# Complexity-ML/complexity-tokenizer

Hardware: AMD Instinct MI355X
Metric: MB/s raw UTF-8 encoded (encode_batch), 50k ByteLevel BPE, 1/2/4/8 MI355X (higher is better)
Workload: dtype u8

## Files before the change

complexity-tokenizer_amd/csrc/seg_lane.h:

```cpp
#pragma once
#include <cstdint>

#if defined(__HIP_DEVICE_COMPILE__)
#define SEG_HD __device__ __forceinline__
#else
#define SEG_HD inline
#endif

namespace seg {

constexpr uint32_t kHi = 0x80808080u;
constexpr uint32_t rep(uint32_t c) { return c * 0x01010101u; }

SEG_HD uint32_t mulhi(uint32_t a, uint32_t b) {
#if defined(__HIP_DEVICE_COMPILE__)
  return __umulhi(a, b);
#else
  return (uint32_t)(((uint64_t)a * b) >> 32);
#endif
}

SEG_HD uint32_t pack8(uint32_t r0, uint32_t r1) {
  const uint32_t c = ((r0 & kHi) >> 4) | (r1 & kHi);
  return mulhi(c, 0x20408100u) & 0xFFu;
}

SEG_HD uint32_t ne7(uint32_t x7, uint32_t c) {
  const uint32_t t = x7 ^ rep(c);
  return (t + 0x7F7F7F7Fu) | t;
}
SEG_HD uint32_t in80(uint32_t x80, uint32_t lo, uint32_t hi) {
  return (x80 - rep(lo)) & ~(x80 - rep(hi + 1));
}

struct Masks {
  uint64_t W, L, N, S, Q, NA;
};
struct Letters {
  uint64_t T1, R, Le, V, LL;
};

SEG_HD Masks ascii_masks(const uint32_t (&x)[16]) {
  uint32_t w[2] = {0, 0}, l[2] = {0, 0}, n[2] = {0, 0}, s[2] = {0, 0}, q[2] = {0, 0}, na[2] = {0, 0};
#pragma unroll
  for (int p = 0; p < 8; p++) {
    const uint32_t a = x[2 * p], b = x[2 * p + 1];
    const uint32_t a7 = a & 0x7F7F7F7Fu, b7 = b & 0x7F7F7F7Fu;
    const uint32_t a80 = a | kHi, b80 = b | kHi;
    const int h = p >> 2, sh = 8 * (p & 3);
    s[h] |= pack8(ne7(a7, ' '), ne7(b7, ' ')) << sh;
    q[h] |= pack8(ne7(a7, '\''), ne7(b7, '\'')) << sh;
    w[h] |= pack8(in80(a80, 9, 13), in80(b80, 9, 13)) << sh;
    l[h] |= pack8(in80(a80 | rep(0x20), 'a', 'z'), in80(b80 | rep(0x20), 'a', 'z')) << sh;
    n[h] |= pack8(in80(a80, '0', '9'), in80(b80, '0', '9')) << sh;
    na[h] |= pack8(a, b) << sh;
  }
  Masks m;
  m.NA = (uint64_t)na[0] | ((uint64_t)na[1] << 32);
  m.S = ~((uint64_t)s[0] | ((uint64_t)s[1] << 32)) & ~m.NA;
  m.Q = ~((uint64_t)q[0] | ((uint64_t)q[1] << 32)) & ~m.NA;
  m.W = (((uint64_t)w[0] | ((uint64_t)w[1] << 32)) | m.S) & ~m.NA;
  m.L = ((uint64_t)l[0] | ((uint64_t)l[1] << 32)) & ~m.NA;
  m.N = ((uint64_t)n[0] | ((uint64_t)n[1] << 32)) & ~m.NA;
  return m;
}

SEG_HD Letters letter_masks(const uint32_t (&x)[16], uint64_t na) {
  uint32_t t1[2] = {0, 0}, r[2] = {0, 0}, e[2] = {0, 0}, v[2] = {0, 0}, ll[2] = {0, 0};
#pragma unroll
  for (int p = 0; p < 8; p++) {
    const uint32_t a7 = x[2 * p] & 0x7F7F7F7Fu, b7 = x[2 * p + 1] & 0x7F7F7F7Fu;
    const int h = p >> 2, sh = 8 * (p & 3);
    t1[h] |= pack8(ne7(a7, 's') & ne7(a7, 't') & ne7(a7, 'm') & ne7(a7, 'd'),
                   ne7(b7, 's') & ne7(b7, 't') & ne7(b7, 'm') & ne7(b7, 'd')) << sh;
    r[h] |= pack8(ne7(a7, 'r'), ne7(b7, 'r')) << sh;
    e[h] |= pack8(ne7(a7, 'e'), ne7(b7, 'e')) << sh;
    v[h] |= pack8(ne7(a7, 'v'), ne7(b7, 'v')) << sh;
    ll[h] |= pack8(ne7(a7, 'l'), ne7(b7, 'l')) << sh;
  }
  auto inv = [&](const uint32_t (&y)[2]) { return ~((uint64_t)y[0] | ((uint64_t)y[1] << 32)) & ~na; };
  return Letters{inv(t1), inv(r), inv(e), inv(v), inv(ll)};
}

SEG_HD uint64_t p1(uint64_t c, uint64_t p) { return (c << 1) | (p >> 63); }
SEG_HD uint64_t p2(uint64_t c, uint64_t p) { return (c << 2) | (p >> 62); }
SEG_HD uint64_t p3(uint64_t c, uint64_t p) { return (c << 3) | (p >> 61); }
SEG_HD uint64_t n1(uint64_t c, uint64_t n) { return (c >> 1) | (n << 63); }
SEG_HD uint64_t n2(uint64_t c, uint64_t n) { return (c >> 2) | (n << 62); }

SEG_HD uint64_t attached(const Masks& c, uint64_t D, uint64_t pW, uint64_t nW, uint64_t nD) {
  const uint64_t E = n1(D, nD);
  return c.S & ~E & ~n1(c.W, nW) & (D | ~p1(c.W, pW));
}

SEG_HD void contractions(const Masks& c, const Letters& lt, uint64_t D, uint64_t A, uint64_t pA, uint64_t pP,
                         uint64_t nL, uint64_t nD, const Letters& nl, uint64_t& C1, uint64_t& C2) {
  const uint64_t E = n1(D, nD);
  const uint64_t P = ~(c.W | c.L | c.N);
  const uint64_t Cb = c.Q & ~E & n1(c.L, nL) & (D | (~p1(P, pP) & ~p1(A, pA)));
  const uint64_t t1 = n1(lt.T1, nl.T1);
  C1 = Cb & t1;
  C2 = Cb & ~t1 & ~n2(D, nD) &
       (((n1(lt.R, nl.R) | n1(lt.V, nl.V)) & n2(lt.Le, nl.Le)) | (n1(lt.LL, nl.LL) & n2(lt.LL, nl.LL)));
}

SEG_HD uint64_t starts(const Masks& c, uint64_t D, uint64_t pW, uint64_t pL, uint64_t pN, uint64_t A, uint64_t pA,
                       uint64_t C1, uint64_t C2, uint64_t pC1, uint64_t pC2) {
  const uint64_t chg = (c.W ^ p1(c.W, pW)) | (c.L ^ p1(c.L, pL)) | (c.N ^ p1(c.N, pN));
  return D | (chg & ~p1(A, pA) & ~p1(C1 | C2, pC1 | pC2)) | (~chg & c.L & (p2(C1, pC1) | p3(C2, pC2)));
}

}
```

complexity-tokenizer_amd/csrc/segment.hip:

```cpp
#include "dev_common.h"
#include "seg_lane.h"

namespace ctok_dev {


__global__ __launch_bounds__(256) void k_tilefirst(const uint64_t* __restrict__ off, uint32_t n_docs, uint32_t n_tiles,
                                                   uint32_t* __restrict__ tfirst, uint32_t* __restrict__ counters) {
  const uint32_t d = blockIdx.x * blockDim.x + threadIdx.x;
  bool empty = false;
  if (d <= n_docs && n_tiles) {
    const uint64_t y = off[d];
    empty = d < n_docs && y == off[d + 1];
    const uint64_t t_lo = d ? (off[d - 1] + 64) / kTile + 1 : 0ull;
    const uint64_t t_hi = min((y + 64) / kTile, (uint64_t)n_tiles - 1);
    for (uint64_t t = t_lo; t <= t_hi && t < t_lo + 64; t++) tfirst[t] = d;
  } else if (d < n_docs) {
    empty = off[d] == off[d + 1];
  }
  const uint64_t me = __ballot(empty);
  if (me && (threadIdx.x & 63) == (uint32_t)__ffsll((unsigned long long)me) - 1)
    atomicAdd(&counters[kCtrEmptyDocs], (uint32_t)__popcll(me));
}

__device__ uint32_t tile_first_search(const uint64_t* off, uint32_t n_docs, uint32_t tile) {
  const uint64_t key = tile ? (uint64_t)tile * kTile - 64 : 0ull;
  uint32_t lo = 0, hi = n_docs;
  while (lo < hi) {
    const uint32_t mid = lo + (hi - lo) / 2;
    if (__builtin_amdgcn_readfirstlane((uint32_t)(off[mid] < key))) lo = mid + 1;
    else hi = mid;
  }
  return lo;
}

__device__ __forceinline__ void clear_words(uint32_t* __restrict__ p, uint64_t n) {
  const uint64_t n4 = n / 4;
  uint4* p4 = reinterpret_cast<uint4*>(p);
  for (uint64_t i = (uint64_t)blockIdx.x * 256 + threadIdx.x; i < n4; i += (uint64_t)gridDim.x * 256)
    p4[i] = make_uint4(0u, 0u, 0u, 0u);
  if (blockIdx.x == 0 && threadIdx.x < n - 4 * n4) p[4 * n4 + threadIdx.x] = 0u;
}

__global__ __launch_bounds__(256) void k_clear(uint32_t* __restrict__ bits, uint64_t n, uint32_t* __restrict__ counters,
                                               uint32_t* __restrict__ tfirst, uint32_t n_tiles) {
  if (bits) clear_words(bits, n);
  for (uint32_t i = blockIdx.x * 256 + threadIdx.x; i < n_tiles; i += gridDim.x * 256) tfirst[i] = ~0u;
  if (blockIdx.x == 0 && counters && threadIdx.x < (uint32_t)kCounterWords) counters[threadIdx.x] = 0u;
}

uint64_t nfc_bits_words(uint64_t n_bytes) { return (n_bytes + 2047) / 2048 + 8; }

hipError_t launch_docstart(const Work& w, hipStream_t s, bool zero_counters, Lx x, Lx x2) {
  const bool nfc = w.nfc_watch == 2;
  const uint64_t n = nfc ? nfc_bits_words(w.n_bytes) : 0;
  const uint64_t work = std::max<uint64_t>(n / 4, w.n_tiles);
  launch_lx(x, k_clear, (unsigned)std::min<uint64_t>((work + 255) / 256 + 1, 8ull * w.n_cus), 256, 0, s,
            nfc ? w.nfc_bits : nullptr, n, zero_counters ? w.counters : nullptr, w.tfirst, w.n_tiles);
  if (w.n_tiles) launch_lx(x2, k_tilefirst, (w.n_docs + 1 + 255) / 256, 256, 0, s, w.doc_off, w.n_docs, w.n_tiles, w.tfirst, w.counters);
  else if (w.n_docs)
    k_tilefirst<<<(w.n_docs + 255) / 256, 256, 0, s>>>(w.doc_off, w.n_docs, 0, w.tfirst, w.counters);
  return hipGetLastError();
}


__device__ __forceinline__ uint32_t piece_probe(const Tables& t, uint4 e, uint32_t h, uint32_t lo, uint32_t hi,
                                                uint32_t n) {
  while (e.z != 0) {
    if (e.x == lo && e.y == hi && e.z == n) return e.w;
    h = (h + 1) & t.piece_mask;
    e = t.piece_tab[h];
  }
  return kNone;
}

__device__ __forceinline__ void seg_wave_sync() {
  __builtin_amdgcn_fence(__ATOMIC_RELEASE, "wavefront");
  __builtin_amdgcn_wave_barrier();
  __builtin_amdgcn_fence(__ATOMIC_ACQUIRE, "wavefront");
}

__device__ __forceinline__ uint32_t select_bit(uint64_t x, uint32_t k) {
  uint32_t pos = 0;
  uint32_t lo = (uint32_t)x, hi = (uint32_t)(x >> 32);
  uint32_t c = __popc(lo);
  uint32_t v = lo;
  if (k >= c) { k -= c; v = hi; pos = 32; }
#pragma unroll
  for (int wdt = 16; wdt >= 1; wdt >>= 1) {
    const uint32_t m = (1u << wdt) - 1u;
    c = __popc(v & m);
    if (k >= c) { k -= c; v >>= wdt; pos += wdt; }
  }
  return pos;
}




#ifdef CTOK_SEG_STAMPS
#define SEG_STAMP(k)                                                                              \
  do {                                                                                            \
    __builtin_amdgcn_sched_barrier(0);                                                            \
    unsigned long long t_;                                                                        \
    asm volatile("s_memtime %0\n\ts_waitcnt lgkmcnt(0)" : "=s"(t_)::"memory");                     \
    __builtin_amdgcn_sched_barrier(0);                                                            \
    if (w.stamps && lane == 0) w.stamps[(size_t)tile * 8 + (k)] = t_;                            \
  } while (0)
#else
#define SEG_STAMP(k) do { } while (0)
#endif
template <bool R16>
__global__ __launch_bounds__(64 * kSegWaves) __attribute__((amdgpu_waves_per_eu(7))) void k_segment(Work w, Tables t) {
  __shared__ uint16_t s_pos_all[kSegWaves][64 * kSegUnroll + 8];
  __shared__ __attribute__((aligned(16))) uint32_t s_text_all[kSegWaves][(kTileWords + 2) * 16 + 8];
  __shared__ uint64_t s_D_all[kSegWaves][64];
  constexpr uint32_t kSegLongCap = 32;
  __shared__ uint64_t s_long_all[kSegWaves][kSegLongCap];
  __shared__ uint8_t s_buf_all[kSegWaves][kSegListBuf];
  const uint32_t lane = threadIdx.x & 63;
  const uint32_t wid = uni(threadIdx.x >> 6);
  const uint32_t tile = uni(blockIdx.x * kSegWaves + wid);
  if (tile >= w.n_tiles) return;
  uint16_t* s_pos = s_pos_all[wid];
  SEG_STAMP(0);
  const uint32_t B = w.n_bytes;
  const uint32_t t0 = tile * kTile;
  const int64_t g = (int64_t)tile * kTileWords - 1 + lane;
  const bool first = lane == 0, last = lane == 63;

  uint32_t x[16];
  uint64_t D, valid;
  {
    const int64_t x0 = g * 64;
    if (x0 >= 0 && x0 + 64 <= (int64_t)B) {
      const uint4* p = reinterpret_cast<const uint4*>(w.text + x0);
#pragma unroll
      for (int k = 0; k < 4; k++) {
        const uint4 v = p[k];
        x[4 * k] = v.x; x[4 * k + 1] = v.y; x[4 * k + 2] = v.z; x[4 * k + 3] = v.w;
      }
      valid = ~0ull;
    } else {
#pragma unroll
      for (int k = 0; k < 16; k++) x[k] = 0;
      valid = 0;
      if (x0 >= 0 && x0 < (int64_t)B) {
        const uint32_t n = B - (uint32_t)x0;
        valid = (1ull << n) - 1;
        for (uint32_t i = 0; i < n; i++) x[i >> 2] |= (uint32_t)w.text[x0 + i] << (8 * (i & 3));
      }
    }
  }
  uint32_t dfirst = uni(w.tfirst[tile]);
  if (dfirst == ~0u) dfirst = tile_first_search(w.doc_off, w.n_docs, tile);
  uint64_t xs0 = ~0ull, ys0 = ~0ull;
  if (dfirst + lane < w.n_docs) {
    xs0 = w.doc_off[dfirst + lane];
    ys0 = w.doc_off[dfirst + lane + 1];
  }
  seg::Masks m = seg::ascii_masks(x);
  {
    uint64_t* s_D = s_D_all[wid];
    s_D[lane] = 0;
    __builtin_amdgcn_fence(__ATOMIC_RELEASE, "wavefront");
    __builtin_amdgcn_wave_barrier();
    const uint64_t base = (uint64_t)t0 - 64;
    const uint64_t lim = (uint64_t)t0 + 4032;
    auto mark = [&](uint64_t xs, uint64_t ys) {
      const bool in = xs < lim;
      if (in && xs != ys) {
        const uint64_t r = xs - base;
        atomicOr((unsigned long long*)&s_D[r >> 6], 1ull << (r & 63));
      }
      return in;
    };
    if (__ballot(mark(xs0, ys0)) == ~0ull) {
      for (uint32_t d = dfirst + 64;; d += 64) {
        const uint32_t i = d + lane;
        uint64_t xs = ~0ull, ys = ~0ull;
        if (i < w.n_docs) {
          xs = w.doc_off[i];
          ys = w.doc_off[i + 1];
        }
        if (__ballot(mark(xs, ys)) != ~0ull) break;
      }
    }
    seg_wave_sync();
    const int64_t x0 = g * 64;
    if (x0 < 0) D = 0;
    else if (x0 >= (int64_t)B) D = ~0ull;
    else D = s_D[lane] | ~valid;
  }
  s_D_all[wid][lane] = D;
  uint32_t* s_all = s_text_all[wid] + 4;
  uint32_t* s_text = s_all + 16;
  if (first && (x[0] & 0xC0u) == 0x80u && g * 64 >= 4)
    s_all[-1] = *reinterpret_cast<const uint32_t*>(w.text + g * 64 - 4);
#pragma unroll
  for (int k = 0; k < 4; k++)
    *reinterpret_cast<uint4*>(s_all + lane * 16 + 4 * k) = make_uint4(x[4 * k], x[4 * k + 1], x[4 * k + 2], x[4 * k + 3]);
  if (last) {
    const int64_t xe = g * 64 + 64;
    uint32_t v = 0;
    if (xe + 4 <= (int64_t)B) {
      v = *reinterpret_cast<const uint32_t*>(w.text + xe);
    } else {
      for (int64_t i = xe; i < (int64_t)B && i < xe + 4; i++) v |= (uint32_t)w.text[i] << (8 * (uint32_t)(i - xe));
    }
    s_all[64 * 16] = v;
  }
  seg_wave_sync();
  SEG_STAMP(1);
  if (m.NA) {
    constexpr int kSegCp = 4;
    bool nfc_bad = false;
    auto set_class = [&](int cl, uint64_t bits) {
      if (cl == 0) m.W |= bits & m.NA;
      else if (cl == 1) m.L |= bits & m.NA;
      else if (cl == 2) m.N |= bits & m.NA;
    };
    uint64_t cont = 0;
#pragma unroll
    for (int k = 0; k < 16; k += 2) {
      const uint32_t c0 = x[k] & ~(x[k] << 1) & seg::kHi, c1 = x[k + 1] & ~(x[k + 1] << 1) & seg::kHi;
      cont |= (uint64_t)seg::pack8(c0, c1) << (4 * k);
    }
    cont &= m.NA;
    const uint64_t lead_cont = cont & ~(cont + 1);
    if (lead_cont) {
      const uint32_t pw = s_all[lane * 16 - 1];
      const int32_t back = ((pw >> 24) & 0xC0u) != 0x80u ? 1 : ((pw >> 16) & 0xC0u) != 0x80u ? 2 : 3;
      const int32_t a = (int32_t)lane * 64 - back;
      const uint32_t v = __builtin_amdgcn_alignbyte(s_all[(a >> 2) + 1], s_all[a >> 2], (uint32_t)a & 3u);
      const uint32_t b0 = v & 255u, b1 = (v >> 8) & 0x3Fu, b2 = (v >> 16) & 0x3Fu, b3 = (v >> 24) & 0x3Fu;
      const int l = u8len((uint8_t)b0);
      const uint32_t c = l == 2 ? ((b0 & 0x1Fu) << 6) | b1
                       : l == 3 ? ((b0 & 0x0Fu) << 12) | (b1 << 6) | b2
                       : l == 4 ? ((b0 & 0x07u) << 18) | (b1 << 12) | (b2 << 6) | b3 : b0;
      const int rc = t.cp_fast ? cp_range_class(c) : -1;
      const int cw = rc >= 0 ? rc : (cls_of(c, t) | (nfc16(t, c) != 0 ? 4 : 0));
      nfc_bad |= (cw & 4) != 0;
      set_class(cw & 3, lead_cont);
    }
    uint64_t leads = m.NA & ~cont;
    while (leads) {
      uint32_t pos[kSegCp], cp[kSegCp], len[kSegCp];
#pragma unroll
      for (int k = 0; k < kSegCp; k++) {
        pos[k] = leads ? (uint32_t)__builtin_ctzll(leads) : 64u;
        leads &= leads ? leads - 1 : 0ull;
      }
#pragma unroll
      for (int k = 0; k < kSegCp; k++) {
        const uint32_t a = lane * 64 + min(pos[k], 63u);
        const uint32_t v = __builtin_amdgcn_alignbyte(s_all[(a >> 2) + 1], s_all[a >> 2], a & 3);
        const uint32_t b0 = v & 255u, b1 = (v >> 8) & 0x3Fu, b2 = (v >> 16) & 0x3Fu, b3 = (v >> 24) & 0x3Fu;
        const int l = u8len((uint8_t)b0);
        len[k] = (uint32_t)l;
        cp[k] = l == 2 ? ((b0 & 0x1Fu) << 6) | b1
              : l == 3 ? ((b0 & 0x0Fu) << 12) | (b1 << 6) | b2
              : l == 4 ? ((b0 & 0x07u) << 18) | (b1 << 12) | (b2 << 6) | b3 : b0;
      }
      int rc[kSegCp];
      uint32_t s1[kSegCp];
#pragma unroll
      for (int k = 0; k < kSegCp; k++) {
        rc[k] = t.cp_fast ? cp_range_class(cp[k]) : -1;
        const bool in = pos[k] < 64 && cp[k] < 0x110000 && rc[k] < 0;
        s1[k] = in && cp[k] < 0x10000 ? (uint32_t)t.cls_bmp[cp[k] >> 1] : 0u;
      }
#pragma unroll
      for (int k = 0; k < kSegCp; k++) {
        if (pos[k] >= 64) continue;
        const uint32_t c = cp[k];
        int cl = 3;
        bool nf = false;
        if (rc[k] >= 0) {
          cl = rc[k];
        } else if (c < 0x80) {
          cl = cls_ascii(c);
        } else if (c < 0x10000) {
          const uint32_t v = s1[k] >> ((c & 1u) * 4);
          cl = (int)(v & 3u);
          nf = (v & 4u) != 0;
        } else if (c < 0x110000) {
          cl = cls_of(c, t);
          nf = nfc16(t, c) != 0;
        }
        nfc_bad |= nf;
        const uint32_t p = pos[k];
        const uint64_t bits = (len[k] >= 64 - p ? ~0ull : ((1ull << len[k]) - 1)) << p;
        set_class(cl, bits);
      }
    }
    if (nfc_bad && w.nfc_watch) {
      atomicOr(&w.counters[kCtrNfcFlag], 1u);
      if (w.nfc_watch == 2 && g >= 0) atomicOr(&w.nfc_bits[g >> 5], 1u << (g & 31));
    }
  }
  SEG_STAMP(2);
  uint64_t pQ = shfl_up64(m.Q);
  if (first) pQ = 0;
  seg::Letters lt{0, 0, 0, 0, 0};
  if (m.Q | (pQ >> 62)) lt = seg::letter_masks(x, m.NA);

  uint64_t st;
  {
    uint64_t pW = shfl_up64(m.W), pL = shfl_up64(m.L), pN = shfl_up64(m.N);
    if (first) pW = pL = pN = 0;
    uint64_t nW = shfl_down64(m.W), nL = shfl_down64(m.L), nD = shfl_down64(D);
    seg::Letters nl{shfl_down64(lt.T1), shfl_down64(lt.R), shfl_down64(lt.Le), shfl_down64(lt.V), shfl_down64(lt.LL)};
    if (last) {
      nW = nL = nD = 0;
      nl = seg::Letters{0, 0, 0, 0, 0};
    }
    const uint64_t A = seg::attached(m, D, pW, nW, nD);
    uint64_t pA = shfl_up64(A);
    if (first) pA = 0;
    uint64_t C1, C2;
    seg::contractions(m, lt, D, A, pA, ~(pW | pL | pN), nL, nD, nl, C1, C2);
    uint64_t pC1 = shfl_up64(C1), pC2 = shfl_up64(C2);
    if (first) pC1 = pC2 = 0;
    st = seg::starts(m, D, pW, pL, pN, A, pA, C1, C2, pC1, pC2) & valid;
    if (last) st &= (1ull << 62) - 1;
    if (!first && !last) {
      const uint64_t gw = (uint64_t)g * 2;
      if (gw < w.n_words) w.pbits[gw] = (uint32_t)st;
      if (gw + 1 < w.n_words) w.pbits[gw + 1] = (uint32_t)(st >> 32);
    }
  }
  const uint32_t nd = uni(wave_sum_full_u32((!first && !last) ? (uint32_t)__popcll(D & valid) : 0u));
  const uint32_t c = (!first && !last) ? (uint32_t)__popcll(st) : 0u;
  const uint32_t inc = wave_incl_scan(c);
  if (!first && !last) w.wpref[(size_t)tile * 64 + lane - 1] = (uint16_t)(inc - c);
  const uint32_t np = lane63(inc);
  const uint32_t tile_end =
      uni((uint32_t)__shfl((int)(st ? (uint32_t)(kTileWords * 64 + __builtin_ctzll(st))
                                    : ((uint64_t)B <= (uint64_t)t0 + kTile + 62 ? (uint32_t)(B - t0) : 0xFFFFu)),
                           63, 64));
  const uint64_t stw = (!first && !last) ? st : 0ull;
  const uint32_t prew = inc - c;
  uint32_t wcur = 1;

  SEG_STAMP(3);
  const bool generic = t.n_at != 0;
  using RecT = typename std::conditional<R16, uint16_t, uint32_t>::type;
  RecT* prec = (RecT*)w.prec + (size_t)tile * kTileSlots;
  uint32_t* pdoc = w.pdoc + (size_t)tile * (kTileSlots / 32);
  uint32_t nm = 0;
  uint32_t n0 = 0, n1 = 0, n2 = 0, n3 = 0;
  uint32_t nlong = 0;
  uint32_t by01 = 0, by2h = 0;
  constexpr int U = kSegUnroll;
  constexpr uint32_t W = 64 * U;
  static_assert(U == 4, "kSegUnroll: 4 (the probes of a round are unrolled by hand)");
  static_assert(kSegListBuf == W && W <= 256, "s_buf: a whole round's pieces, one byte each");
  uint8_t* s_buf = s_buf_all[wid];
  uint32_t cnt = 0;
  auto flush = [&]() __attribute__((always_inline)) {
    const uint64_t below = lanemask_lt();
    for (uint32_t p0 = 0; p0 < cnt; p0 += 64) {
      const uint32_t i = p0 + lane, ord = nm + i;
      uint32_t bsl = 0, bn = 0;
      uint32_t cl = 4;
      if (i < cnt) {
        const uint32_t k = s_buf[i];
        const uint32_t a = s_pos[k], el = s_pos[k + 1];
        bsl = seg_mark_start(a);
        cl = seg_mark_class(a);
        bn = el == 0xFFFFu ? 0u : seg_mark_start(el) - bsl;
      }
      uint64_t m0 = __ballot(cl == 0);
      if (n0 + (uint32_t)__popcll(m0) > w.k0) {
        if (cl == 0 && n0 + (uint32_t)__popcll(m0 & below) >= w.k0) cl = 3;
        m0 = __ballot(cl == 0);
      }
      const uint32_t e = list_entry(bsl, ord, bn);
      {
        const uint64_t m1 = __ballot(cl == 1), m2 = __ballot(cl == 2);
        const uint64_t m3 = __ballot(cl == 6);
        if (cl == 0) w.list0[(size_t)tile * w.k0 + n0 + __popcll(m0 & below)] = e;
        if (cl == 1) w.list1[(size_t)tile * kCap1 + n1 + __popcll(m1 & below)] = e;
        if (cl == 2) w.list2[(size_t)tile * kCap2 + n2 + __popcll(m2 & below)] = e;
        if (cl == 6) w.list3[(size_t)tile * kCap3 + n3 + __popcll(m3 & below)] = e;
        by01 += cl == 0 ? bn : cl == 1 ? bn << 16 : 0u;
        by2h += cl == 2 ? bn : 0u;
        n0 += __popcll(m0);
        n1 += __popcll(m1);
        n2 += __popcll(m2);
        n3 += __popcll(m3);
      }
      const uint64_t lm = __ballot(cl == 3);
      const uint64_t le = (uint64_t)(t0 + bsl) | ((uint64_t)ord << 32) | ((uint64_t)bn << 44);
      if (lm && nlong + (uint32_t)__popcll(lm) <= kSegLongCap) {
        if (cl == 3) s_long_all[wid][nlong + __popcll(lm & below)] = le;
        nlong += (uint32_t)__popcll(lm);
      } else if (lm) {
        const uint32_t leader = __ffsll((unsigned long long)lm) - 1;
        uint32_t b = 0;
        if (lane == leader) b = atomicAdd(&w.counters[kCtrLong], (uint32_t)__popcll(lm));
        b = __builtin_amdgcn_readlane(b, leader);
        const uint32_t li = b + __popcll(lm & below);
        if (cl == 3 && li < w.long_cap) w.long_list[li] = le;
        if (lane == leader && b + __popcll(lm) > w.long_cap) atomicOr(&w.counters[kCtrOverflow], 1u);
      }
    }
    nm += cnt;
    cnt = 0;
  };
  for (uint32_t j0 = 0; j0 < np; j0 += W) {
    for (uint32_t wb = wcur;; wb += 32) {
      const uint32_t wl = wb + (lane >> 1), src = min(wl, 63u);
      const uint32_t lo32 = (uint32_t)__shfl((int)(uint32_t)stw, (int)src, 64);
      const uint32_t hi32 = (uint32_t)__shfl((int)(uint32_t)(stw >> 32), (int)src, 64);
      const uint32_t pw = (uint32_t)__shfl((int)prew, (int)src, 64);
      const bool hi = (lane & 1) != 0;
      uint32_t bits = wl <= (uint32_t)kTileWords ? (hi ? hi32 : lo32) : 0u;
      uint32_t k = pw + (hi ? (uint32_t)__popc(lo32) : 0u);
      if (k > j0 + W || k + (uint32_t)__popc(bits) <= j0) bits = 0;
      const uint32_t pos0 = (wl - 1) * 64 + (hi ? 32u : 0u);
      while (bits) {
        const uint32_t b = (uint32_t)__builtin_ctz(bits);
        if (k >= j0 && k <= j0 + W) s_pos[k - j0] = (uint16_t)(pos0 + b);
        bits &= bits - 1u;
        k++;
      }
      const uint32_t wn = wb + 32;
      if (wn > (uint32_t)kTileWords || uni(__builtin_amdgcn_readlane(prew, wn)) > j0 + W) break;
    }
    {
      const uint64_t inw = __ballot(lane >= wcur && lane <= (uint32_t)kTileWords && prew <= j0 + W);
      if (inw) wcur = 63u - (uint32_t)__builtin_clzll(inw);
    }

    if (lane == 0 && np <= j0 + W) s_pos[np - j0] = (uint16_t)tile_end;
    seg_wave_sync();
    uint32_t sl[U], n[U], cls[U], plo[U], phi[U], h[U], doc[U];
#pragma unroll
    for (int u = 0; u < U; u++) {
      const uint32_t j = j0 + 64 * u + lane;
      sl[u] = 0;
      n[u] = 0;
      doc[u] = 0;
      cls[u] = 4;
      if (j < np) {
        sl[u] = s_pos[64 * u + lane];
        doc[u] = (uint32_t)(s_D_all[wid][(sl[u] >> 6) + 1] >> (sl[u] & 63)) & 1u;
        const uint32_t el = s_pos[64 * u + lane + 1];
        if (el == 0xFFFFu || el - sl[u] > (generic ? (uint32_t)kShortMax : (uint32_t)kMedMax)) {
          cls[u] = 3;
        } else {
          n[u] = el - sl[u];
          cls[u] = generic ? 0 : n[u] > 32 ? 6 : n[u] > 16 ? 2 : n[u] > 8 ? 1 : 5;
        }
      }
      const uint32_t a = sl[u] >> 2, sh = sl[u] & 3;
      const uint32_t d0 = s_text[a], d1 = s_text[a + 1], d2 = s_text[a + 2];
      const uint32_t w0 = __builtin_amdgcn_alignbyte(d1, d0, sh), w1 = __builtin_amdgcn_alignbyte(d2, d1, sh);
      const uint32_t nn = n[u];
      plo[u] = nn >= 4 ? w0 : w0 & ((1u << (8 * nn)) - 1u);
      phi[u] = nn >= 8 ? w1 : nn <= 4 ? 0u : w1 & ((1u << (8 * (nn - 4))) - 1u);
      h[u] = cls[u] == 5 ? piece_hash(plo[u], phi[u], nn) & t.piece_mask : t.piece_mask + 1;
    }
    uint32_t hitv[U];
#define CTOK_PROBE_LOAD(u) const uint4 e##u = t.piece_tab[h[u]];
#define CTOK_PROBE_USE(u) hitv[u] = piece_probe(t, e##u, h[u], plo[u], phi[u], n[u]);
    CTOK_PROBE_LOAD(0) CTOK_PROBE_LOAD(1) CTOK_PROBE_LOAD(2) CTOK_PROBE_LOAD(3)
    CTOK_PROBE_USE(0) CTOK_PROBE_USE(1) CTOK_PROBE_USE(2) CTOK_PROBE_USE(3)
#undef CTOK_PROBE_LOAD
#undef CTOK_PROBE_USE
#pragma unroll
    for (int u = 0; u < U; u++) {
      const uint32_t j = j0 + 64 * u + lane;
      uint32_t rec = kRecMerged32;
      if (cls[u] == 5) {
        const bool hit = hitv[u] != kNone;
        rec = hit ? hitv[u] : kRecMerged32;
        by2h += hit ? 0x10000u : 0u;
        cls[u] = hit ? 4u : 0u;
      }
      if (j < np) {
        prec[j] = (RecT)rec;
      }
      const uint64_t dm = __ballot(doc[u] != 0);
      if (lane == 0 && j0 + 64 * u < np)
        *reinterpret_cast<uint2*>(pdoc + ((j0 + 64 * u) >> 5)) = make_uint2((uint32_t)dm, (uint32_t)(dm >> 32));
    }
    seg_wave_sync();
#pragma unroll
    for (int u = 0; u < U; u++) {
      const uint64_t mm = __ballot(cls[u] != 4);
      if (cls[u] != 4) {
        s_pos[64 * u + lane] = (uint16_t)seg_mark(sl[u], cls[u]);
        s_buf[cnt + (uint32_t)__popcll(mm & lanemask_lt())] = (uint8_t)(64 * u + lane);
      }
      cnt += (uint32_t)__popcll(mm);
    }
    seg_wave_sync();
    flush();
    seg_wave_sync();
  }
  if (nlong) {
    uint32_t b = 0;
    if (lane == 0) b = atomicAdd(&w.counters[kCtrLong], nlong);
    b = __builtin_amdgcn_readfirstlane(b);
    seg_wave_sync();
    if (lane < nlong && b + lane < w.long_cap) w.long_list[b + lane] = s_long_all[wid][lane];
    if (lane == 0 && b + nlong > w.long_cap) atomicOr(&w.counters[kCtrOverflow], 1u);
  }
  SEG_STAMP(4);
  by01 = wave_sum_full_u32(by01);
  by2h = wave_sum_full_u32(by2h);
  const uint32_t by0 = by01 & 0xFFFFu, by1 = by01 >> 16, by2 = by2h & 0xFFFFu, hits = by2h >> 16;
  if (lane == 0) {
    w.tile_tok[tile] = hits;
    w.tile_doc[tile] = nd;
    w.tile_np[tile] = np;
    w.tregion[tile] = make_uint2(by0 | ((by0 + by1) << 16), by0 + by1 + by2);
  }
  if (lane < kNumClasses)
    w.rend[(size_t)lane * w.n_tiles + tile] = lane == 0 ? 0u : lane == 1 ? by0 : lane == 2 ? by0 + by1 : by0 + by1 + by2;
  if (lane < kNumClasses)
    w.tcls[(size_t)lane * w.n_tiles + tile] = lane == 0 ? n0 : lane == 1 ? n1 : lane == 2 ? n2 : n3;
  if (lane == 0 && n2) w.counters[kCtrAnyMid] = 1;
  if (lane == 0 && n3) w.counters[kCtrAnyC3] = 1;
  if (n3 && w.c3_max) {
    const uint32_t sh = tile & (kC3Shards - 1), cap = w.c3_max / kC3Shards;
    uint32_t b = 0;
    if (lane == 0) b = atomicAdd(&w.counters[kNumCounters + sh], n3);
    b = __builtin_amdgcn_readfirstlane(b);
    for (uint32_t j = lane; j < n3; j += 64)
      if (b + j < cap) w.c3q[(size_t)sh * cap + b + j] = (tile << 7) | j;
  }
  SEG_STAMP(5);
#ifdef CTOK_SEG_STAMPS
  if (w.stamps && lane == 0) w.stamps[(size_t)tile * 8 + 6] = np;
#endif
}

hipError_t launch_segment(const Work& w, const Tables& t, hipStream_t s, Lx x) {
  const uint32_t grid = (w.n_tiles + kSegWaves - 1) / kSegWaves;
  if (w.n_tiles && w.rec16) launch_lx(x, k_segment<true>, grid, 64 * kSegWaves, 0, s, w, t);
  else if (w.n_tiles) launch_lx(x, k_segment<false>, grid, 64 * kSegWaves, 0, s, w, t);
  return hipGetLastError();
}

}
```

Measured before the change: 179,200.

## Pack byte masks with udot4 and build per-piece doc bitmap up front

Replaces the mulhi-based byte-to-bit packing with two chained v_dot4 unsigned byte dot products, with the shift folded into a pack8_at helper. Separately, the per-piece document-start bitmap is now built once per tile: each lane ORs bits for doc-starting pieces into LDS via popcount ranking, and the bitmap is written out before the main piece loop. This removes the per-iteration LDS lookup and ballot store from the hot loop. The trade is extra LDS atomics, an additional wave sync, and reuse of the s_D buffer, which depends on D no longer being needed from LDS later.

Result: faster. 182,800 (median of 6 runs) (+2.0%).

```diff
diff --git a/complexity-tokenizer_amd/csrc/seg_lane.h b/complexity-tokenizer_amd/csrc/seg_lane.h
--- a/complexity-tokenizer_amd/csrc/seg_lane.h
+++ b/complexity-tokenizer_amd/csrc/seg_lane.h
@@ -12,17 +12,22 @@
 constexpr uint32_t kHi = 0x80808080u;
 constexpr uint32_t rep(uint32_t c) { return c * 0x01010101u; }
 
-SEG_HD uint32_t mulhi(uint32_t a, uint32_t b) {
+SEG_HD uint32_t dot4(uint32_t a, uint32_t b, uint32_t c) {
 #if defined(__HIP_DEVICE_COMPILE__)
-  return __umulhi(a, b);
+  return __builtin_amdgcn_udot4(a, b, c, false);
 #else
-  return (uint32_t)(((uint64_t)a * b) >> 32);
+  for (int k = 0; k < 32; k += 8) c += ((a >> k) & 255u) * ((b >> k) & 255u);
+  return c;
 #endif
 }
 
-SEG_HD uint32_t pack8(uint32_t r0, uint32_t r1) {
-  const uint32_t c = ((r0 & kHi) >> 4) | (r1 & kHi);
-  return mulhi(c, 0x20408100u) & 0xFFu;
+SEG_HD uint32_t pack8_hi(uint32_t r0, uint32_t r1) {
+  return dot4(r1 & kHi, 0x80402010u, dot4(r0 & kHi, 0x08040201u, 0u));
+}
+SEG_HD uint32_t pack8(uint32_t r0, uint32_t r1) { return pack8_hi(r0, r1) >> 7; }
+SEG_HD uint32_t pack8_at(uint32_t r0, uint32_t r1, int sh) {
+  const uint32_t v = pack8_hi(r0, r1);
+  return sh >= 7 ? v << (sh - 7) : v >> (7 - sh);
 }
 
 SEG_HD uint32_t ne7(uint32_t x7, uint32_t c) {
@@ -48,12 +53,12 @@
     const uint32_t a7 = a & 0x7F7F7F7Fu, b7 = b & 0x7F7F7F7Fu;
     const uint32_t a80 = a | kHi, b80 = b | kHi;
     const int h = p >> 2, sh = 8 * (p & 3);
-    s[h] |= pack8(ne7(a7, ' '), ne7(b7, ' ')) << sh;
-    q[h] |= pack8(ne7(a7, '\''), ne7(b7, '\'')) << sh;
-    w[h] |= pack8(in80(a80, 9, 13), in80(b80, 9, 13)) << sh;
-    l[h] |= pack8(in80(a80 | rep(0x20), 'a', 'z'), in80(b80 | rep(0x20), 'a', 'z')) << sh;
-    n[h] |= pack8(in80(a80, '0', '9'), in80(b80, '0', '9')) << sh;
-    na[h] |= pack8(a, b) << sh;
+    s[h] |= pack8_at(ne7(a7, ' '), ne7(b7, ' '), sh);
+    q[h] |= pack8_at(ne7(a7, '\''), ne7(b7, '\''), sh);
+    w[h] |= pack8_at(in80(a80, 9, 13), in80(b80, 9, 13), sh);
+    l[h] |= pack8_at(in80(a80 | rep(0x20), 'a', 'z'), in80(b80 | rep(0x20), 'a', 'z'), sh);
+    n[h] |= pack8_at(in80(a80, '0', '9'), in80(b80, '0', '9'), sh);
+    na[h] |= pack8_at(a, b, sh);
   }
   Masks m;
   m.NA = (uint64_t)na[0] | ((uint64_t)na[1] << 32);
@@ -71,12 +76,12 @@
   for (int p = 0; p < 8; p++) {
     const uint32_t a7 = x[2 * p] & 0x7F7F7F7Fu, b7 = x[2 * p + 1] & 0x7F7F7F7Fu;
     const int h = p >> 2, sh = 8 * (p & 3);
-    t1[h] |= pack8(ne7(a7, 's') & ne7(a7, 't') & ne7(a7, 'm') & ne7(a7, 'd'),
-                   ne7(b7, 's') & ne7(b7, 't') & ne7(b7, 'm') & ne7(b7, 'd')) << sh;
-    r[h] |= pack8(ne7(a7, 'r'), ne7(b7, 'r')) << sh;
-    e[h] |= pack8(ne7(a7, 'e'), ne7(b7, 'e')) << sh;
-    v[h] |= pack8(ne7(a7, 'v'), ne7(b7, 'v')) << sh;
-    ll[h] |= pack8(ne7(a7, 'l'), ne7(b7, 'l')) << sh;
+    t1[h] |= pack8_at(ne7(a7, 's') & ne7(a7, 't') & ne7(a7, 'm') & ne7(a7, 'd'),
+                      ne7(b7, 's') & ne7(b7, 't') & ne7(b7, 'm') & ne7(b7, 'd'), sh);
+    r[h] |= pack8_at(ne7(a7, 'r'), ne7(b7, 'r'), sh);
+    e[h] |= pack8_at(ne7(a7, 'e'), ne7(b7, 'e'), sh);
+    v[h] |= pack8_at(ne7(a7, 'v'), ne7(b7, 'v'), sh);
+    ll[h] |= pack8_at(ne7(a7, 'l'), ne7(b7, 'l'), sh);
   }
   auto inv = [&](const uint32_t (&y)[2]) { return ~((uint64_t)y[0] | ((uint64_t)y[1] << 32)) & ~na; };
   return Letters{inv(t1), inv(r), inv(e), inv(v), inv(ll)};
diff --git a/complexity-tokenizer_amd/csrc/seg_route_hd.h b/complexity-tokenizer_amd/csrc/seg_route_hd.h
--- /dev/null
+++ b/complexity-tokenizer_amd/csrc/seg_route_hd.h
@@ -0,0 +1,20 @@
+#pragma once
+#include <cstdint>
+
+#if defined(__HIPCC__)
+#define SEG_RT_HD __host__ __device__ __forceinline__
+#else
+#define SEG_RT_HD inline
+#endif
+
+namespace seg {
+
+template <class F>
+SEG_RT_HD void doc_pieces(uint64_t st, uint64_t D, uint32_t prew, F set) {
+  for (uint64_t m = D & st; m; m &= m - 1ull) {
+    const uint64_t below = (m & (0ull - m)) - 1ull;
+    set(prew + (uint32_t)__builtin_popcountll(st & below));
+  }
+}
+
+}
diff --git a/complexity-tokenizer_amd/csrc/segment.hip b/complexity-tokenizer_amd/csrc/segment.hip
--- a/complexity-tokenizer_amd/csrc/segment.hip
+++ b/complexity-tokenizer_amd/csrc/segment.hip
@@ -1,5 +1,6 @@
 #include "dev_common.h"
 #include "seg_lane.h"
+#include "seg_route_hd.h"
 
 namespace ctok_dev {
 
@@ -159,6 +160,7 @@
     ys0 = w.doc_off[dfirst + lane + 1];
   }
   seg::Masks m = seg::ascii_masks(x);
+  asm volatile("" : "+v"(m.W), "+v"(m.L), "+v"(m.N), "+v"(m.S), "+v"(m.Q), "+v"(m.NA));
   {
     uint64_t* s_D = s_D_all[wid];
     s_D[lane] = 0;
@@ -191,7 +193,6 @@
     else if (x0 >= (int64_t)B) D = ~0ull;
     else D = s_D[lane] | ~valid;
   }
-  s_D_all[wid][lane] = D;
   uint32_t* s_all = s_text_all[wid] + 4;
   uint32_t* s_text = s_all + 16;
   if (first && (x[0] & 0xC0u) == 0x80u && g * 64 >= 4)
@@ -341,12 +342,26 @@
   const uint64_t stw = (!first && !last) ? st : 0ull;
   const uint32_t prew = inc - c;
   uint32_t wcur = 1;
+  uint32_t* pdoc = w.pdoc + (size_t)tile * (kTileSlots / 32);
+  {
+    static_assert(kTileSlots == 64 * 64, "the pdoc bitmap of a tile: s_D's 64 u64 words");
+    uint32_t dl = lane;
+    asm volatile("" : "+v"(dl));
+    uint64_t* s_doc = s_D_all[wid];
+    s_doc[dl] = 0;
+    seg_wave_sync();
+    seg::doc_pieces(stw, D, prew, [&](uint32_t j) { atomicOr((uint32_t*)s_doc + (j >> 5), 1u << (j & 31)); });
+    seg_wave_sync();
+    if (lane * 64 < np) {
+      const uint64_t dm = s_doc[dl];
+      *reinterpret_cast<uint2*>(pdoc + 2 * lane) = make_uint2((uint32_t)dm, (uint32_t)(dm >> 32));
+    }
+  }
 
   SEG_STAMP(3);
   const bool generic = t.n_at != 0;
   using RecT = typename std::conditional<R16, uint16_t, uint32_t>::type;
   RecT* prec = (RecT*)w.prec + (size_t)tile * kTileSlots;
-  uint32_t* pdoc = w.pdoc + (size_t)tile * (kTileSlots / 32);
   uint32_t nm = 0;
   uint32_t n0 = 0, n1 = 0, n2 = 0, n3 = 0;
   uint32_t nlong = 0;
@@ -435,17 +450,15 @@
 
     if (lane == 0 && np <= j0 + W) s_pos[np - j0] = (uint16_t)tile_end;
     seg_wave_sync();
-    uint32_t sl[U], n[U], cls[U], plo[U], phi[U], h[U], doc[U];
+    uint32_t sl[U], n[U], cls[U], plo[U], phi[U], h[U];
 #pragma unroll
     for (int u = 0; u < U; u++) {
       const uint32_t j = j0 + 64 * u + lane;
       sl[u] = 0;
       n[u] = 0;
-      doc[u] = 0;
       cls[u] = 4;
       if (j < np) {
         sl[u] = s_pos[64 * u + lane];
-        doc[u] = (uint32_t)(s_D_all[wid][(sl[u] >> 6) + 1] >> (sl[u] & 63)) & 1u;
         const uint32_t el = s_pos[64 * u + lane + 1];
         if (el == 0xFFFFu || el - sl[u] > (generic ? (uint32_t)kShortMax : (uint32_t)kMedMax)) {
           cls[u] = 3;
@@ -482,9 +495,6 @@
       if (j < np) {
         prec[j] = (RecT)rec;
       }
-      const uint64_t dm = __ballot(doc[u] != 0);
-      if (lane == 0 && j0 + 64 * u < np)
-        *reinterpret_cast<uint2*>(pdoc + ((j0 + 64 * u) >> 5)) = make_uint2((uint32_t)dm, (uint32_t)(dm >> 32));
     }
     seg_wave_sync();
 #pragma unroll
```
